# NWC-CUAHSI-Summer-Institute/LGAR-py

Hardware: AMD Instinct MI355X
Metric: column-timesteps/sec (higher is better)
Workload: dtype f32

## Files before the change

lgar_py_amd/csrc/lgar_column.hpp:

```cpp
#pragma once
#include "lgar_geff.hpp"

namespace lgar {

template <typename R> struct Glob {
  R dt_h, initial_psi, pdm, wp_psi, frozen;
  R giuh[LGAR_GMAX];
  int nint, nsub, ng, bottom_mode, closed_form;
  long long iter_cap;
};

#define LGAR_COOP_GROUPS 16
template <typename S, int FMAX, int STRIDE = WAVE> struct FrontsView {
  S *base;
  unsigned char *fl;
  __device__ __forceinline__ S &Z(int i) const { return base[(0 * FMAX + i) * STRIDE]; }
  __device__ __forceinline__ S &TH(int i) const { return base[(1 * FMAX + i) * STRIDE]; }
  __device__ __forceinline__ S &PS(int i) const { return base[(2 * FMAX + i) * STRIDE]; }
  __device__ __forceinline__ S &DZ(int i) const { return base[(3 * FMAX + i) * STRIDE]; }
  __device__ __forceinline__ unsigned char &flag(int i) const { return fl[i * STRIDE]; }
  __device__ __forceinline__ int layer(int i) const { return fl[i * STRIDE] & 0x7f; }
  __device__ __forceinline__ bool bottom(int i) const { return (fl[i * STRIDE] & LGAR_FLAG_BOTTOM) != 0; }
  __device__ __forceinline__ void set_flag(int i, int layer, bool bottom) const {
    fl[i * STRIDE] = (unsigned char)(layer | (bottom ? LGAR_FLAG_BOTTOM : 0));
  }
  __device__ __forceinline__ void copy(int dst, int src) const {
    Z(dst) = Z(src); TH(dst) = TH(src); PS(dst) = PS(src); DZ(dst) = DZ(src);
    fl[dst * STRIDE] = fl[src * STRIDE];
  }
};

constexpr int MODE_LITERAL = 0, MODE_FAST = 1, MODE_MIXED = 3, MODE_COOP = 4, MODE_MIXED_COOP = 6;

template <typename S, int MODE> struct ModeTraits : ScalarKind<S> {
  using K = ScalarKind<S>;
  static constexpr bool literal = MODE == MODE_LITERAL;
  static constexpr bool mixed = MODE == MODE_MIXED || MODE == MODE_MIXED_COOP;
  static constexpr bool coop = MODE == MODE_COOP || MODE == MODE_MIXED_COOP;
  static constexpr bool mixed_f64 = mixed && K::plain_f64;
  static constexpr bool coop_f64 = coop && K::plain_f64;
  static constexpr int pol = (literal && K::f64) ? POL_LIBRARY : (!literal && K::plain_f32) ? POL_RCP32 : mixed_f64 ? POL_MIXED : POL_LEAN;
  static constexpr int stride = coop ? LGAR_COOP_GROUPS : WAVE;
  static constexpr bool giuh_mem = MODE == MODE_MIXED && !K::dual;
  static constexpr bool late_forcing_sums = MODE == MODE_MIXED;
  static constexpr bool fused_walk = !literal && !coop;
};

template <typename S, int NL, int FMAX, int MODE> struct Column {
  using R = real_t<S>;
  using M = ModeTraits<S, MODE>;
  static constexpr int POL = M::pol;
  const ColParams<S, NL> &P;
  const LGAR_KARG Glob<R> *G;
  FrontsView<S, FMAX, M::stride> F;
  int nf;
  int status;
  S ponded_water, previous_precip, ending_volume;
  S giuh_q[LGAR_GMAX];
  static constexpr int DEAD = LGAR_ST_BOTTOM | LGAR_ST_OVERFLOW | LGAR_ST_STRUCT;
  R *giuh_mem = nullptr;
  size_t giuh_stride = 0;
  bool giuh_live = false;
  S k_deepest;
  bool new_front_frozen;
  S memo_theta, memo_g;
  int memo_layer = -1;
  unsigned near_sat_fronts = 0u;
  S post_mass;
  bool post_mass_valid = false;
  bool post_event = false;
  bool psi_rewritten = false;
  S aet_psi_wp_memo;
  bool aet_psi_wp_known = false;
  bool count_geff = false;
  int share_lanes = 0;
  R *xchg = nullptr;
  int coop_rank = 0;
  int cap = FMAX;
  S a_precip, a_pet, a_aet, a_infil, a_runoff, a_perc, a_giuh, a_disch;

  __device__ Column(const ColParams<S, NL> &p, const LGAR_KARG Glob<R> *g, const FrontsView<S, FMAX, M::stride> &f) : P(p), G(g), F(f) {}

  __device__ __forceinline__ S cum_at(int k) const { return sel<S, NL>(P.cum, k); }
  __device__ __forceinline__ S capillary_drive(const LayerK<S> &lk, S theta1, S theta2, int site = 0, CoopRiders *riders = nullptr) {
    (void)site; (void)riders;
    LGAR_MEASURE_POINT(NOGEFF, lk, theta1, theta2)
    LGAR_COUNT_GEFF_CALL(site)
    LGAR_MEASURE_POINT(DUP_GEFF, lk, theta1, theta2)
    if constexpr (M::literal && M::f64) {
      return G->closed_form ? geff_closed<S, POL>(lk, theta1, theta2) : geff_literal<S, POL>(lk, theta1, theta2, G->nint);
    }
    if constexpr (M::dual && M::f64 && !M::literal) {
      if (share_lanes >= 2 && !G->closed_form) return geff_fused<S>(lk, theta1, theta2, G->nint, xchg, share_lanes);
    }
    if constexpr (M::coop_f64 && !M::mixed) {
      if (share_lanes > 1 && !G->closed_form) return geff_fused<S>(lk, theta1, theta2, G->nint, xchg, share_lanes, coop_rank, riders);
    }
    if constexpr (M::coop_f64 && M::mixed) {
      if (share_lanes > 1 && !G->closed_form)
        return geff_mixed_coop(val(lk.alpha), val(lk.n), val(lk.m), val(lk.inv_m), val(lk.inv_n), val(lk.ksat), val(lk.te), val(lk.tr),
                               theta1, theta2, G->nint, xchg, share_lanes, coop_rank);
    }
    if constexpr (M::mixed_f64) {
      if (!G->closed_form)
        return geff_mixed(val(lk.alpha), val(lk.n), val(lk.m), val(lk.inv_m), val(lk.inv_n), val(lk.ksat), val(lk.te), val(lk.tr),
                          theta1, theta2, G->nint);
    }
#ifndef LGAR_NO_F32_RARE_GEFF
    if constexpr (M::plain_f32 && !M::literal) {
      if (site != 1 && !G->closed_form)
        return geff_f32_rare(lk.alpha, lk.n, lk.m, lk.inv_m, lk.inv_n, lk.te, lk.tr, theta1, theta2, G->nint);
    }
#endif
    return G->closed_form ? geff_closed<S, POL>(lk, theta1, theta2) : geff(lk, theta1, theta2, G->nint);
  }
  __device__ __forceinline__ double capillary_drive_fronts(const LayerK<double> &lk, double theta1, double theta2, double psi1,
                                                           double psi2, double &kr_end) {
    LGAR_MEASURE_POINT(NOGEFF_FRONTS, lk, theta1, theta2, kr_end)
    LGAR_COUNT_GEFF_CALL(1)
    if constexpr (M::coop && M::mixed) {
      if (share_lanes > 1) return geff_mixed_heads<true>(lk, theta1, theta2, psi1, psi2, G->nint, kr_end, xchg, share_lanes, coop_rank);
    }
    return geff_mixed_heads(lk, theta1, theta2, psi1, psi2, G->nint, kr_end);
  }
  __device__ __forceinline__ S cum_prev(int k) const {
    S r = S(R(0.0));
#pragma unroll
// ... 1016 lines not shown
      const LayerK<S> lk = pick(P, k);
      LGAR_COUNT_GEFF_CALL(1)
      LGAR_COUNT_GEFF_CALL(1)
      double kr_mine;
      const S g_mine = geff_mixed_heads<true>(lk, F.TH(im + 1), F.TH(im), F.PS(im + 1), F.PS(im), G->nint, kr_mine, tab2, hl, r2);
      tab2[0] = g_mine;
      tab2[1] = kr_mine;
#pragma unroll
      for (int j = 0; j < NL - 1; j++)
        if (j < kmax) {
          const LayerK<S> lj = pick_static(P, j);
          const S tl = theta_from_h<S, POL>(lj, F.PS(im));
          tab2[2 + j] = k_from_se<S, POL>(lj, se_from_theta(lj, tl));
        }
      lds_exchange_point();
      S g2[2];
      R kr2[2], kk[2][NL];
#pragma unroll
      for (int h = 0; h < 2; h++) {
        g2[h] = xchg[h * 64];
        kr2[h] = xchg[h * 64 + 1];
#pragma unroll
        for (int j = 0; j < NL - 1; j++) kk[h][j] = xchg[h * 64 + 2 + j];
      }
      lds_exchange_point();
#pragma unroll
      for (int h = 0; h < 2; h++) {
        const int f = h ? ib : ia;
        const int kf = h ? kb : ka;
        const LayerK<S> lf = pick(P, kf);
        const S g = g2[h];
        S ki = lf.ksat * kr2[h];
        if (f == 0 && new_front_frozen) ki = ki * G->frozen;
        if (is_nan(val(g))) status |= LGAR_ST_NAN;
        const S delta_theta = F.TH(f) - F.TH(f + 1);
        S dzdt;
        if (kf == 0) {
          dzdt = dv<POL>(S(R(1.0)), delta_theta) * (dv<POL>(lf.ksat * (g + h_p), F.Z(f)) + ki);
        } else {
          S den = S(R(0.0)) + dv<POL>(F.Z(f) - cum_prev(kf), ki);
#pragma unroll
          for (int j = 0; j < NL - 1; j++)
            if (j < kf) {
              S pt = (j != 0) ? P.cum[(j > 0) ? j - 1 : 0] : S(R(0.0));
              den = den + dv<POL>(P.cum[j] - pt, S(kk[h][j]));
            }
          dzdt = dv<POL>(S(R(1.0)), delta_theta) * (dv<POL>(F.Z(f), den) + dv<POL>(lf.ksat * (g + h_p), F.Z(f)));
        }
        F.DZ(f) = dzdt;
      }
    }
  }

  __device__ __forceinline__ void calc_dzdt(S h_p) {
    int i = -1;
    if constexpr (M::coop_f64 && M::mixed) {
      if (share_lanes >= 4 && !G->closed_form) i = calc_dzdt_pairs_mixed(h_p);
    }
    if constexpr (M::coop_f64 && !M::mixed) {
      if (share_lanes >= LGAR_COOP_PAIR_LANES && !G->closed_form) i = calc_dzdt_pairs(h_p);
    }
    for (;;) {
      bool found = false;
      while (!found && ++i < nf - 1) {
        if (F.bottom(i)) { F.DZ(i) = S(R(0.0)); continue; }
        const bool top = F.layer(i) == 0;
        if (top && val(F.TH(i + 1)) > val(F.TH(i))) status |= LGAR_ST_THETA_ORDER;
        if (val(F.TH(i) - F.TH(i + 1)) > R(0.0)) found = true;
        else F.DZ(i) = S(R(0.0));
      }
      if (any_lane(found) == 0ull) break;
      LGAR_MEASURE_POINT(CLK, 10)
      if (found) {
        const int k = F.layer(i);
        const LayerK<S> lk = pick(P, k);
        S theta_1 = F.TH(i + 1), theta_2 = F.TH(i);
        S delta_theta = F.TH(i) - F.TH(i + 1);
        S g, ki;
        bool fronts_done = false;
        if constexpr (M::mixed_f64) {
          if (!G->closed_form) {
            double kr_end;
            g = capillary_drive_fronts(lk, theta_1, theta_2, F.PS(i + 1), F.PS(i), kr_end);
            ki = lk.ksat * kr_end;
            if (i == 0 && new_front_frozen) ki = ki * G->frozen;
            fronts_done = true;
          }
        }
        CoopRiders riders;
        if constexpr (M::coop_f64 && !M::mixed) {
          if (!G->closed_form && share_lanes >= 5 + k) {
            const int e = coop_rank - 5;
            LayerK<S> le = lk;
            S th_e = F.TH(i);
            if (k > 0) {
#pragma unroll
              for (int j = 0; j < NL - 1; j++) {
                const bool mine = (e == j) && (j < k);
                le.alpha = choose(mine, P.alpha[j], le.alpha); le.n = choose(mine, P.n[j], le.n); le.m = choose(mine, P.m[j], le.m);
                le.inv_m = choose(mine, P.inv_m[j], le.inv_m); le.ksat = choose(mine, P.ksat[j], le.ksat);
                le.te = choose(mine, P.te[j], le.te); le.tr = choose(mine, P.tr[j], le.tr);
              }
              const S tl = theta_from_h<S, POL>(le, F.PS(i));
              th_e = choose(e >= 0 && e < k, tl, th_e);
            }
            riders.n = 1 + k;
            riders.l = le;
            riders.se = se_from_theta(le, th_e);
#pragma unroll
            for (int q = 0; q < LGAR_LMAX; q++) riders.k[q] = R(1.0);
            g = capillary_drive(lk, theta_1, theta_2, 1, &riders);
            ki = riders.k[0];
            if (i == 0 && new_front_frozen) ki = ki * G->frozen;
            fronts_done = true;
          }
        }
        LGAR_MEASURE_POINT(F32_HEADS_FROM_PSI, lk, i, g, ki, fronts_done)
        if (!fronts_done) {
          g = capillary_drive(lk, theta_1, theta_2, 1);
          ki = front_k(i, lk);
#ifndef LGAR_NO_DZDT_MEMO
          if constexpr (M::plain_f32 && !M::literal) {
            if (same_bits(theta_2, lk.te) && (i == 0 || F.layer(i - 1) != k)) { memo_theta = theta_1; memo_g = g; memo_layer = k; }
          }
#endif
        }
        if (is_nan(val(g))) status |= LGAR_ST_NAN;
        S dzdt;
        if (k == 0) {
          dzdt = dv<POL>(S(R(1.0)), delta_theta) * (dv<POL>(lk.ksat * (g + h_p), F.Z(i)) + ki);
        } else {
          S den = S(R(0.0)) + dv<POL>(F.Z(i) - cum_prev(k), ki);
#pragma unroll
          for (int j = 0; j < NL - 1; j++)
            if (j < k) {
              const LayerK<S> lj = pick_static(P, j);
              S kl;
              bool rode = false;
              if constexpr (M::coop_f64 && !M::mixed) {
                if (riders.n > 0) { kl = riders.k[1 + j]; rode = true; }
              }
              if (!rode) {
                S tl = theta_from_h<S, POL>(lj, F.PS(i));
                kl = k_from_se<S, POL>(lj, se_from_theta(lj, tl));
              }
              S pt = (j != 0) ? P.cum[(j > 0) ? j - 1 : 0] : S(R(0.0));
              den = den + dv<POL>(P.cum[j] - pt, kl);
            }
          dzdt = dv<POL>(S(R(1.0)), delta_theta) * (dv<POL>(F.Z(i), den) + dv<POL>(lk.ksat * (g + h_p), F.Z(i)));
        }
        F.DZ(i) = dzdt;
        LGAR_MEASURE_POINT(CLK, 17)
      }
    }
  }

  __device__ __forceinline__ S calc_dry_depth() {
    const LayerK<S> l0 = pick_static(P, 0);
    S delta_theta = l0.te - F.TH(0);
    S tau = G->dt_h * l0.ksat / delta_theta;
    S g = capillary_drive(l0, F.TH(0), l0.te, 2);
    if (is_nan(val(g))) status |= LGAR_ST_NAN;
    S dry = R(0.5) * (tau + sq(tau * tau + R(4.0) * tau * g));
    return mn(P.cum[0], dry);
  }

  __device__ __forceinline__ void create_surficial_front(S dry_depth, S &ponded, S &infiltration) {
    if (nf >= cap) { status |= LGAR_ST_OVERFLOW; return; }
    const LayerK<S> l0 = pick_static(P, 0);
    S cur_theta = F.TH(0);
    S delta_theta = l0.te - cur_theta;
    S theta_new;
    bool to_bottom = false;
    if (val(dry_depth * delta_theta) > val(ponded)) {
      infiltration = ponded;
      theta_new = mn((cur_theta + ponded / dry_depth), l0.te);
      ponded = S(R(0.0));
    } else {
      infiltration = dry_depth * delta_theta;
      ponded = ponded - (dry_depth * delta_theta);
      theta_new = l0.te;
      to_bottom = !(val(dry_depth) < val(P.cum[0]));
    }
    for (int j = nf; j > 0; j--) F.copy(j, j - 1);
    nf++;
    F.Z(0) = dry_depth;
    F.TH(0) = theta_new;
    F.set_flag(0, 0, to_bottom);
    F.PS(0) = h_from_se<S, POL>(l0, se_from_theta(l0, theta_new));
    new_front_frozen = true;
    F.DZ(0) = S(R(0.0));
  }

  __device__ __forceinline__ void insert_water(int fdd, S precip, S &ponded, S &infiltration, S &runoff) {
    const R dt = G->dt_h;
    S h_p = (ponded - precip) * dt;
    if (val(h_p) < R(0.0)) h_p = S(R(0.0));
    const int kfp = F.layer(fdd);
    int lo, len;
    range_of(kfp, lo, len);
    const int nxt_i = lo + 1;
    if (nxt_i >= nf && (nf != NL || G->bottom_mode == 0)) { status |= LGAR_ST_STRUCT; return; }
    const LayerK<S> lk = pick(P, kfp);
    S g = S(R(0.0));
    if (nf != NL) {
      const S theta_1 = F.TH(nxt_i < nf ? nxt_i : nf - 1);
      bool hit = memo_layer == kfp && same_bits(theta_1, memo_theta);
      if constexpr (M::dual) {
        if (share_lanes >= 2) {
          const bool value_hit = memo_layer == kfp && val(theta_1) == val(memo_theta);
          if (any_lane(value_hit && !hit) != 0ull) hit = false;
        }
      }
      if (hit) {
        g = memo_g;
      } else {
        g = capillary_drive(lk, theta_1, lk.te, 3);
        memo_theta = theta_1; memo_g = g; memo_layer = kfp;
      }
    }
    if (is_nan(val(g))) status |= LGAR_ST_NAN | LGAR_ST_NEGBASE;
    S f_p;
    if (kfp == 0) {
      f_p = P.ksat[0] * (R(1.0) + dv<POL>(g + h_p, F.Z(fdd)));
    } else {
      S fd_ksat = lk.ksat * G->frozen;
      S bottom_sum = dv<POL>(F.Z(fdd) - cum_prev(kfp), fd_ksat);
      bottom_sum = bottom_sum + dv<POL>(P.cum[0] - R(0.0), P.ksat[0] * G->frozen);
#pragma unroll
      for (int j = 1; j < NL - 1; j++)
        if (j < kfp) {
          const LayerK<S> lj = pick_static(P, j);
          S tl = theta_from_h<S, POL>(lj, F.PS(fdd));
          S kl = k_from_se<S, POL>(lj, se_from_theta(lj, tl));
          bottom_sum = bottom_sum + dv<POL>(P.cum[j] - P.cum[j - 1], kl);
        }
      f_p = dv<POL>(F.Z(fdd), bottom_sum) + dv<POL>((g + h_p) * fd_ksat, F.Z(fdd));
    }
    S pond_temp = ponded - f_p * dt;
    if (val(pond_temp) < R(0.0)) pond_temp = S(R(0.0));
    S fp_cm = f_p * dt;
    if (G->pdm > R(0.0)) {
      if (val(pond_temp) < G->pdm) {
        infiltration = mn(ponded, fp_cm);
        ponded = ponded - infiltration;
      } else if (val(pond_temp) > G->pdm) {
        ponded = S(G->pdm);
        infiltration = fp_cm;
      }
      S r = pond_temp - G->pdm;
      runoff = (val(r) > R(0.0)) ? r : S(R(0.0));
    } else {
      infiltration = mn(ponded, fp_cm);
      S r = ponded - infiltration;
      ponded = S(G->pdm);
      runoff = (val(r) > R(0.0)) ? r : S(R(0.0));
    }
  }

  __device__ __forceinline__ void init_state() {
    nf = NL;
    status = 0;
    new_front_frozen = false;
#pragma unroll
    for (int k = 0; k < NL; k++) {
      const LayerK<S> lk = pick_static(P, k);
      F.Z(k) = P.cum[k];
      F.TH(k) = theta_from_h<S, POL>(lk, S(G->initial_psi));
      F.PS(k) = S(G->initial_psi);
      if (k == NL - 1) k_deepest = k_from_se<S, POL>(lk, se_from_theta(lk, F.TH(k)));
      F.DZ(k) = S(R(0.0));
      F.set_flag(k, k, true);
    }
    ponded_water = previous_precip = S(R(0.0));
#pragma unroll
    for (int i = 0; i < LGAR_GMAX; i++) giuh_q[i] = S(R(0.0));
    ending_volume = mass_balance();
    drain();
  }

  __device__ __forceinline__ void drain() {
    a_precip = a_pet = a_aet = a_infil = a_runoff = a_perc = a_giuh = a_disch = S(R(0.0));
  }

  __device__ __forceinline__ void forward(S precip, S pet) {
    const R dt = G->dt_h;
    if (is_nan(val(precip)) || is_nan(val(pet))) status |= LGAR_ST_NAN;
    S ending_volume_sub = ending_volume;
    for (int sub = 0; sub < G->nsub; sub++) {
      if (status & DEAD) return;
      new_front_frozen = false;
      post_mass_valid = false;
      S precip_sub = precip * dt;
      S pet_sub = pet * dt;
      S ponded_depth_sub = precip_sub + ponded_water;
      S ponded_water_sub = S(R(0.0)), runoff_sub = S(R(0.0)), infiltration_sub = S(R(0.0)), AET_sub = S(R(0.0));
      const bool create = (val(previous_precip) == R(0.0)) && (val(precip_sub) > R(0.0)) && (val(ponded_water) == R(0.0));
      LGAR_MEASURE_POINT(CLK, 0)
      LGAR_MEASURE_POINT(DUP_FDD)
      const int fdd = free_drainage_front();
      const bool saturated = val(F.TH(0)) >= val(P.te[0]);
      if (val(pet) > R(0.0)) {
        if (!aet_psi_wp_known) {
          aet_psi_wp_memo = aet_psi_wp<S, POL>(pick_static(P, 0), G->wp_psi);
          aet_psi_wp_known = true;
        }
        AET_sub = aet_from_psi_wp<S, POL>(pet, dt, F.PS(0), aet_psi_wp_memo);
      }
      if constexpr (!M::late_forcing_sums) {
        a_precip = a_precip + precip_sub;
        a_pet = a_pet + ((val(pet_sub) > R(0.0)) ? pet_sub : S(R(0.0)));
      }
      const bool inserting = !create && val(ponded_depth_sub) > R(0.0);
      LGAR_MEASURE_POINT(CLK, 1)
      if (inserting) {
        LGAR_ABLATABLE(INSERT, insert_water(fdd, precip_sub, ponded_depth_sub, infiltration_sub, runoff_sub);)
        a_infil = a_infil + infiltration_sub;
        a_runoff = a_runoff + runoff_sub;
        ponded_water_sub = ponded_depth_sub;
      }
      LGAR_MEASURE_POINT(CLK, 2)
      if (!create || !saturated) {
        S perc_sub = S(R(0.0));
        LGAR_ABLATABLE(MOVE, perc_sub = move_wetting_front(create ? S(R(0.0)) : infiltration_sub, AET_sub, ending_volume_sub, fdd);)
        if (!create) a_perc = a_perc + perc_sub;
      }
      if (__builtin_expect(create && !saturated, 0)) {
        S dry_depth = calc_dry_depth();
        create_surficial_front(dry_depth, ponded_depth_sub, infiltration_sub);
        a_infil = a_infil + infiltration_sub;
        post_mass_valid = false;
      }
      if (!inserting) {
        if (val(ponded_depth_sub) < G->pdm) {
          runoff_sub = S(R(0.0));
          ponded_water_sub = ponded_depth_sub;
          ponded_depth_sub = S(R(0.0));
        } else {
          runoff_sub = ponded_depth_sub - G->pdm;
          ponded_depth_sub = S(G->pdm);
          ponded_water_sub = ponded_depth_sub;
          a_runoff = a_runoff + runoff_sub;
        }
      }
      LGAR_MEASURE_POINT(CLK, 5)
      LGAR_ABLATABLE(DZDT, calc_dzdt(ponded_depth_sub);)
      LGAR_MEASURE_POINT(CLK, 6)
      LGAR_MEASURE_POINT(DUP_DZDT, ponded_depth_sub)
      LGAR_MEASURE_POINT(DUP_MB, ending_volume_sub)
      if constexpr (M::fused_walk) {
        if (__builtin_expect(!post_mass_valid, 0)) post_mass = mass_balance();
        ending_volume_sub = post_mass;
      } else {
        ending_volume_sub = mass_balance();
      }
      LGAR_MEASURE_POINT(CLK, 7)
      previous_precip = precip_sub;
      ending_volume = ending_volume_sub;
      if constexpr (M::late_forcing_sums) {
        a_precip = a_precip + precip_sub;
        a_pet = a_pet + ((val(pet_sub) > R(0.0)) ? pet_sub : S(R(0.0)));
      }
      a_aet = a_aet + AET_sub;
      ponded_water = ponded_water_sub;
      if constexpr (M::giuh_mem) {
        if (giuh_live || val(runoff_sub) > R(0.0)) {
          const int ng = G->ng;
          S q[LGAR_GMAX];
#pragma unroll
// ... 44 lines not shown
```

lgar_py_amd/csrc/lgar_forward_body.hpp:

```cpp
#pragma once
#include "lgar_column.hpp"

namespace lgar {

template <typename R> struct KArgs {
  int N, T, F;
  int Nf, Fg;
  int coop;
  unsigned *ticket;
  int chain_first, chain_last;
  const unsigned *pending_in;
  unsigned *pending_out;
  const R *alpha, *n, *ksat, *theta_e, *theta_r, *thick;
  R *depth, *theta, *psi, *k, *dzdt;
  uint8_t *flags;
  int32_t *nf;
  R *scalars;
  R *totals;
  const R *precip, *pet;
  R *series[LGAR_NACC];
  double *basin;
  const R *weights;
  unsigned basin_mask;
  int32_t *status;
// ... 262 lines not shown
    bool active = (t >= t_begin) && (t < t_stop_at.get());
    if (active && !a.chain_last && col.nf + a.G.nsub > FMAX) {
      active = false;
      t_stop_at.set(t);
    }
    if (any_lane(active) == 0ull) continue;
    if (active) col.forward(precip, pet);
    LGAR_MEASURE_POINT(BALLAST_TOUCH)
    if constexpr (AHEAD) {
      settle_load(precip_ahead);
      settle_load(pet_ahead);
    }
    const R acc[LGAR_NACC] = {col.a_precip, col.a_pet, col.a_aet, col.a_infil, col.a_runoff,
                              col.a_perc, col.a_giuh, col.a_disch, col.ponded_water, col.ending_volume};
    if (active && leader) {
#pragma unroll
      for (int j = 0; j < LGAR_NACC; j++)
        if (series_mask & (1u << j)) a.series[j][o] = acc[j];
    }
    LGAR_MEASURE_POINT(CLK, 18)
    if (basin_on) {
      const double w = active ? wgt : 0.0;
#pragma unroll
      for (int j = 0; j < LGAR_NACC; j++)
        if (a.basin_mask & (1u << j)) {
          const double s = wave_sum(w * (double)acc[j]);
          if (lane == 0) {
            if constexpr (PARK) atomic_add_uniform(&a.basin[(size_t)j * T + t], s);
            else atomic_add(&a.basin[(size_t)j * T + t], s);
          }
        }
    }
    if (active) {
#pragma unroll
      for (int j = 0; j < 7; j++) {
        if (j == 5 && a.G.bottom_mode == 0) continue;
        const int row = sum_row<SR>(j);
        if (row >= 0) lds.sums[row][slot] = lds.sums[row][slot] + acc[j];
        else tot[j] = tot[j] + acc[j];
      }
      col.drain();
    }
    LGAR_MEASURE_POINT(CLK, 21)
  }
  LGAR_MEASURE_POINT(BALLAST_FOLD, col)
  ap = launder(ap);
  const LGAR_KARG KArgs<R> &z = *ap;
  if (z.counters != nullptr) {
    const double calls = wave_sum((double)((unsigned)col.status >> LGAR_ST_STEP_SHIFT));
    if (lane == 0 && calls > 0.0) {
      if constexpr (PARK) atomic_add_uniform(&z.counters[0], (unsigned long long)calls);
      else atomic_add(&z.counters[0], (unsigned long long)calls);
    }
  }
  col.status &= LGAR_ST_FAULT_MASK;
  const int t_stop = t_stop_at.get();
  if (t_begin >= z.T) return;
  if (!leader) return;
  if (z.pending_out != nullptr) {
    const unsigned long long m = any_lane(t_stop >= 0 && t_stop < z.T);
    if (m != 0ull && first_active_lane()) {
      if constexpr (PARK) atomic_add_uniform(z.pending_out, (unsigned)__builtin_popcountll(m));
      else atomic_add(z.pending_out, (unsigned)__builtin_popcountll(m));
    }
  }
  int word = col.status;
  if (t_stop >= 0 && t_stop < z.T) word |= LGAR_ST_RESUME | (int)((unsigned)t_stop << LGAR_ST_STEP_SHIFT);
  if (t_stop <= t_begin) {
    z.status[c] = word;
    if (z.call_sums != nullptr && z.chain_first) {
#pragma unroll
      for (int j = 0; j < 8; j++) z.call_sums[j * N + c] = R(0);
      z.call_sums[8 * N + c] = col.ponded_water;
      z.call_sums[9 * N + c] = col.ending_volume;
    }
    return;
  }
  store_state<R, NL, FMAX, MODE>(z, c, col, nf_before, word);
#pragma unroll
  for (int j = 0; j < 7; j++)
    if (sum_row<SR>(j) >= 0) tot[j] = lds.sums[sum_row<SR>(j)][slot];
  tot[7] = tot[6];
#pragma unroll
  for (int j = 0; j < 8; j++) z.totals[j * N + c] = z.totals[j * N + c] + tot[j];
  z.totals[8 * N + c] = col.ponded_water;
  z.totals[9 * N + c] = col.ending_volume;
  if (z.call_sums != nullptr) {
    const bool add = !z.chain_first;
#pragma unroll
    for (int j = 0; j < 8; j++) z.call_sums[j * N + c] = add ? z.call_sums[j * N + c] + tot[j] : tot[j];
    z.call_sums[8 * N + c] = col.ponded_water;
    z.call_sums[9 * N + c] = col.ending_volume;
  }
}

}
```

lgar_py_amd/csrc/lgar_geff.hpp:

```cpp
#pragma once
#include "lgar_vg.hpp"

namespace lgar {

#define LGAR_COOP_TAB 128
#define LGAR_COOP_TAB_ROW 130
#define LGAR_COOP_PAIR_LANES 12
#ifndef LGAR_DEVSIM
template <int W>
__device__ __forceinline__ void geff_coop_node_rounds(const LayerK<double> &l, double nm1, double half_m, double k_sat1, double k_first,
                                                      double hdh, int nint, int lanes, double *tab, int r) {
  const int stride = W * lanes;
  for (int first = 0; first < nint; first += stride) {
    double h[W], k[W];
    bool ok[W];
#pragma unroll
    for (int u = 0; u < W; u++) {
      const int j = first + r + u * lanes;
      ok[u] = (r < lanes) && (j < nint);
      h[u] = tab[ok[u] ? j : 0];
    }
#pragma unroll
    for (int u = 0; u < W; u++) k[u] = geff_node(l, nm1, half_m, h[u]);
#pragma unroll
// ... 283 lines not shown
    const f32x2 t = __builtin_elementwise_fma(-P, (SR) * (SR), one2);          \
    (TT) = t * t;                                                              \
  }
  int it = 0;
  for (; it + 1 < safe_pairs; it += 2) {
    const f32x2 xa = __builtin_elementwise_fma(ja, dx2, x02);
    const f32x2 xb = __builtin_elementwise_fma(ja + two2, dx2, x02);
    ja = ja + four2;
    f32x2 sa, ta, sb, tb;
    LGAR_GEFF_PAIR(xa, sa, ta)
    acc = __builtin_elementwise_fma(sa, ta, acc);
    LGAR_GEFF_PAIR(xb, sb, tb)
    accb = __builtin_elementwise_fma(sb, tb, accb);
  }
  if (it < safe_pairs) {
    const f32x2 x = __builtin_elementwise_fma(ja, dx2, x02);
    f32x2 sr, tt;
    LGAR_GEFF_PAIR(x, sr, tt)
    acc = __builtin_elementwise_fma(sr, tt, acc);
    it++;
  }
  for (; it < pairs; it++) {
    const float j0 = float(2 * it + 1);
    const f32x2 j2 = {j0, j0 + 1.0f};
    const f32x2 x = __builtin_elementwise_fma(j2, dx2, x02);
    f32x2 sr, tt;
    LGAR_GEFF_PAIR(x, sr, tt)
    sr.x = (x.x < xcut) ? ksat1 : sr.x;
    tt.x = (x.x < xcut) ? 1.0f : tt.x;
    sr.y = (x.y < xcut) ? ksat1 : sr.y;
    tt.y = (x.y < xcut) ? 1.0f : tt.y;
    if (it & 1) accb = __builtin_elementwise_fma(sr, tt, accb);
    else acc = __builtin_elementwise_fma(sr, tt, acc);
  }
  acc = acc + accb;
  float sum = acc.x + acc.y;
  if (M & 1) sum += node(__builtin_fmaf(float(M), dx, x0));
#ifndef LGAR_NO_GEFF_ENDS
  float k0, kn;
  {
    const f32x2 xe = {x0, l.alpha * h_f};
    f32x2 sr, tt;
    LGAR_GEFF_PAIR(xe, sr, tt)
    sr.x = (xe.x < xcut) ? ksat1 : sr.x;
    tt.x = (xe.x < xcut) ? 1.0f : tt.x;
    sr.y = (xe.y < xcut) ? ksat1 : sr.y;
    tt.y = (xe.y < xcut) ? 1.0f : tt.y;
    const f32x2 ke = sr * tt;
    k0 = ke.x; kn = ke.y;
  }
#else
  const float k0 = node(x0), kn = node(l.alpha * h_f);
#endif
#undef LGAR_GEFF_PAIR
  if (kn_out != nullptr) *kn_out = kn;
  return fabsf((0.5f * dh) * ((k0 + kn) + 2.0f * sum));
}
template <> __device__ __forceinline__ float geff<float>(const LayerK<float> &l, float theta1, float theta2, int nint) {
  const float se_i = se_from_theta(l, theta1);
  const float se_f = se_from_theta(l, theta2);
  const float inv_alpha = 1.0f / l.alpha;
#ifndef LGAR_NO_GEFF_ENDS
  const float ni = -l.inv_m;
  const float la = lg2(se_i), lb = lg2(se_f);
  const float pa = ex2(ni * la), pb = ex2(ni * lb);
  float ba = pa - 1.0f, bb = pb - 1.0f;
  if (fabsf(ba) <= 1e-8f) ba = ba + 1e-12f;
  if (fabsf(bb) <= 1e-8f) bb = bb + 1e-12f;
  const float ua = lg2(ba), ub = lg2(bb);
  const float oa = ex2(l.inv_n * ua), ob = ex2(l.inv_n * ub);
  return geff_f32_from_heads(l, inv_alpha * oa, inv_alpha * ob, nint);
#else
  auto head = [&](float se) {
    float base = pw(se, -l.inv_m) - 1.0f;
    if (fabsf(base) <= 1e-8f) base = base + 1e-12f;
    return inv_alpha * pw(base, l.inv_n);
  };
  return geff_f32_from_heads(l, head(se_i), head(se_f), nint);
#endif
}
__device__ __attribute__((noinline)) float geff_f32_rare(float alpha, float n, float m, float inv_m, float inv_n, float te, float tr,
                                                         float theta1, float theta2, int nint) {
  const LayerK<float> l{alpha, n, m, inv_m, inv_n, 1.0f, te, tr};
  return geff<float>(l, theta1, theta2, nint);
}
template <> __device__ __forceinline__ double geff<double>(const LayerK<double> &l, double t1, double t2, int nint) {
  return geff_fused<double>(l, t1, t2, nint);
}

#define LGAR_LOG2_1EM12 -39.863137138648355
__device__ __forceinline__ void mixed_end(const LayerK<double> &l, double se, double &h, double &kr) {
  const double q = lg2e(se) * l.inv_m;
  const double C = ex2e(q);
  const double omc = 1.0 - C;
  const bool k_nudged = fabs(omc) <= 1e-8;
  const double bk = k_nudged ? omc + 1e-12 : omc;
  const double u = (omc == 0.0) ? LGAR_LOG2_1EM12 : lg2e(bk);
  const double t = 1.0 - ex2e(l.m * u);
  kr = sqrt(se) * (t * t);
  const double bh = omc / C;
  const bool h_nudged = fabs(bh) <= 1e-8;
  double lbh = (omc == 0.0) ? u : u - q;
  if (any_lane((k_nudged || h_nudged) && omc != 0.0) != 0ull) {
    const double own = lg2e(h_nudged ? bh + 1e-12 : bh);
    lbh = ((k_nudged || h_nudged) && omc != 0.0) ? own : lbh;
  }
  h = (1.0 / l.alpha) * ex2e(lbh * l.inv_n);
}
template <bool COOPERATE = false>
__device__ __forceinline__ double geff_mixed_core(const LayerK<double> &l, double h_i, double h_f, double k0, double kn_own, double ksat1,
                                                  int nint, double *tab = nullptr, int lanes = 0, int r = 0) {
  (void)tab; (void)lanes; (void)r;
  const float ksat1f = (float)ksat1;
  const double dh = (h_f - h_i) / double(nint);
  const double x0 = l.alpha * h_i, dx = l.alpha * dh, xcut = 0.1 * l.alpha;
  const double hmd = -0.5 * l.m;
  const float hm = (float)hmd, hm_lo = (float)(hmd - (double)hm);
  const int M = nint - 1;
  const int pairs = M >> 1;
  const double inv_ndx = 1.0 / -dx;
  const double jf = (x0 - xcut) * inv_ndx - 1.5;
  int safe = (jf > 0.0) ? ((jf < double(M)) ? int(jf) : M) : 0;
  safe >>= 1;
  int safe_pairs = pairs;
  if (!COOPERATE && any_lane(safe < pairs) != 0ull) {
    safe_pairs = 0;
    for (int bit = 64; bit; bit >>= 1) {
      const int cand = safe_pairs + bit;
      if (cand <= pairs && any_lane(safe < cand) == 0ull) safe_pairs = cand;
    }
  }
  const float xcutf = (float)xcut;
  const float nf = (float)l.n, nf_lo = (float)(l.n - (double)nf), mmf = (float)(-l.m), mmf_lo = (float)(-l.m - (double)mmf);
  const f32x2 n2 = {nf, nf}, nl2 = {nf_lo, nf_lo}, hm2 = {hm, hm}, hml2 = {hm_lo, hm_lo}, one2 = {1.0f, 1.0f};
  const f32x2 ln2_2 = {0.693147181f, 0.693147181f}, c2_2 = {0.240226507f, 0.240226507f}, c3_2 = {0.0555041087f, 0.0555041087f};
  const f32x2 c4_2 = {0.00961812911f, 0.00961812911f}, c5_2 = {0.00133335581f, 0.00133335581f};
  const f32x2 mm2 = {mmf, mmf}, mml2 = {mmf_lo, mmf_lo}, ilog2 = {1.44269504f, 1.44269504f}, two_ilog2 = {2.88539008f, 2.88539008f};
  const f32x2 half2 = {0.5f, 0.5f};
// ... 253 lines not shown
```

lgar_py_amd/csrc/lgar_measure.hpp:

```cpp
#pragma once
#ifdef LGAR_NO_F32_REUSE
#define LGAR_NO_DZDT_MEMO
#define LGAR_NO_F32_RARE_GEFF
#define LGAR_NO_GEFF_ENDS
#endif

__device__ __forceinline__ float opaque(float x) { asm volatile("" : "+v"(x)); return x; }
__device__ __forceinline__ double opaque(double x) { asm volatile("" : "+v"(x)); return x; }

#define LGAR_MEASURE_POINT(NAME, ...) LGAR_POINT_##NAME(__VA_ARGS__)
#define LGAR_ABLATABLE(NAME, ...) LGAR_STMT_##NAME(__VA_ARGS__)

#ifdef LGAR_ABL_NOINSERT
#define LGAR_STMT_INSERT(...)
#else
#define LGAR_STMT_INSERT(...) __VA_ARGS__
#endif
#ifdef LGAR_ABL_NOMOVE
#define LGAR_STMT_MOVE(...)
#else
#define LGAR_STMT_MOVE(...) __VA_ARGS__
#endif
#ifdef LGAR_ABL_NODZDT
#define LGAR_STMT_DZDT(...)
#else
#define LGAR_STMT_DZDT(...) __VA_ARGS__
#endif

#ifdef LGAR_ABL_NOGEFF
#define LGAR_POINT_NOGEFF(lk, theta1, theta2) return theta1 * theta2 + lk.alpha;
#else
#define LGAR_POINT_NOGEFF(lk, theta1, theta2)
#endif
#ifdef LGAR_ABL_NOGEFF
#define LGAR_POINT_NOGEFF_FRONTS(lk, theta1, theta2, kr) { kr = theta1; return theta1 * theta2 + lk.alpha; }
#else
#define LGAR_POINT_NOGEFF_FRONTS(lk, theta1, theta2, kr)
#endif
#ifdef LGAR_COUNT_SITE
#define LGAR_COUNT_IF_SITE(site) if (site == LGAR_COUNT_SITE)
#else
#define LGAR_COUNT_IF_SITE(site)
#endif
#ifdef LGAR_COUNT_MAXLANES
#define LGAR_COUNT_IF_SPARSE if (__builtin_popcountll(any_lane(true)) <= LGAR_COUNT_MAXLANES)
#else
#define LGAR_COUNT_IF_SPARSE
#endif
#ifdef LGAR_COUNT_LANES
#define LGAR_COUNT_WHO count_geff
#else
#define LGAR_COUNT_WHO (count_geff && first_active_lane())
#endif
#define LGAR_COUNT_GEFF_CALL(site) \
  LGAR_COUNT_IF_SITE(site) LGAR_COUNT_IF_SPARSE { if (LGAR_COUNT_WHO) status += (1 << LGAR_ST_STEP_SHIFT); }
#ifdef LGAR_DUP_GEFF
#define LGAR_POINT_DUP_GEFF(lk, theta1, theta2)                                                    \
// ... 141 lines not shown
```

lgar_py_amd/engine.py:

```python
import ctypes as C

import torch

from . import _capi
from ._capi import ACC_NAMES, GMAX, LMAX, LMIN, NACC, NSCAL, LgarError

BASIN_SCRATCH_BYTES = 8 << 30
PARAMS = ("alpha", "n", "ksat", "theta_e", "theta_r", "thickness")
SETTINGS = dict(dt_h=1.0, num_subcycles=1, initial_psi=2000.0, ponded_depth_max=0.0, wilting_point_psi=15495.0,
                frozen_factor=1.0, nint=120, giuh_ordinates=(0.06, 0.51, 0.28, 0.12, 0.03), dtype=torch.float64,
                device="cuda:0", iter_cap=0, search_mode=1, bottom_mode=0, use_closed_form_G=False, front_slots=None,
                geff_precision="native", forward_lanes=0, basin_scratch_bytes=BASIN_SCRATCH_BYTES)
_DIMS_SETTINGS = ("dt_h", "num_subcycles", "initial_psi", "ponded_depth_max", "wilting_point_psi", "frozen_factor", "nint",
                  "giuh_ordinates", "iter_cap", "search_mode", "bottom_mode", "use_closed_form_G", "forward_lanes")


def _require_gpu(device):
    if not torch.cuda.is_available():
        raise LgarError("no ROCm GPU visible: the LGAR engine has no CPU fallback (device=%s)" % (device,))


def _ptr(t):
    return None if t is None else t.data_ptr()

# ... 204 lines not shown
            st["d_in"].copy_(h_in, non_blocking=True)
            _capi.check(self.lib.lgar_forward(*st["args"], self._dt, C.c_void_p(stream.cuda_stream)), "lgar_forward")
            st["h_out"].copy_(st["d_out"], non_blocking=True)
            st["h_status"].copy_(self.status, non_blocking=True)
            stream.synchronize()
        return st["h_out"][:NACC], st["h_out"][NACC], st["h_out"][NACC + 1], st["h_status"]

    def raise_for_status(self, status_host):
        if bool((status_host != 0).any()):
            self.check_status()

    def tangent(self, direction, precip, pet, w_runoff=None, w_perc=None, want_series=False, forcing_group=1, share=0):
        prep = lambda t: None if t is None else torch.as_tensor(t).to(self.device, self.dtype).contiguous()
        precip, pet = self._forcing(precip, pet, forcing_group)
        w_runoff, w_perc = prep(w_runoff), prep(w_perc)
        share = int(share)
        if share != 0 and (not 2 <= share <= 32 or self.N % share != 0):
            raise LgarError("share must be 0 or 2..32 (with n_columns a multiple of it)")
        if share:
            for t in (self.alpha, self.n, self.ksat, self.theta_e, self.theta_r, self.thickness):
                gw = t.reshape(t.shape[0], -1, share)
                if not bool((gw == gw[:, :, :1]).all()):
                    raise LgarError("share=%d needs identical soil parameters within each group of %d columns" % (share, share))
            if forcing_group % share != 0 and precip.shape[1] != 1:
                raise LgarError("share=%d needs the columns of a group to read the same forcing column (forcing_group a "
                                "multiple of it, or one forcing column for all)" % share)
        self.dims.tangent_share = int(share)
        for nm, w in (("w_runoff", w_runoff), ("w_perc", w_perc)):
            if w is not None and w.shape != precip.shape:
                raise LgarError("%s must be [T, N] like the forcing; got %s" % (nm, tuple(w.shape)))
        T = precip.shape[0]
        dirs = {k: prep(direction.get(k)) for k in ("alpha", "n", "ksat")}
        for k, v in dirs.items():
            if v is not None and tuple(v.shape) != (self.L, self.N):
                raise LgarError("direction[%r] must be [L, N]" % k)
        dstruct = _capi.LgarParams(_ptr(dirs["alpha"]), _ptr(dirs["n"]), _ptr(dirs["ksat"]), None, None, None)
        grad = torch.zeros(self.N, dtype=self.dtype, device=self.device)
        ser = self._new_series(T, self.N, dtype=self.dtype, device=self.device) if want_series else None
        st = torch.zeros(self.N, dtype=torch.int32, device=self.device)
        tickets = torch.zeros(_capi.NTICKETS, dtype=torch.int32, device=self.device)
        fo = _capi.LgarForcing(precip.data_ptr(), pet.data_ptr())
        self._call("forward_tangent", C.byref(self.dims), C.byref(self._params), C.byref(dstruct), C.byref(fo), _ptr(w_runoff),
                   _ptr(w_perc), grad.data_ptr(), _ptr(ser), st.data_ptr(), counters=tickets)
        return grad, ser, st

    def cooperating_lanes(self):
        return int(self.lib.lgar_cooperating_lanes(C.byref(self.dims), self._dt))

    def geff_wave_calls(self, reset=True):
        n = int(self.counters[0].item())
        if reset:
            self.counters.zero_()
        return n

    def check_status(self):
        st = self.status
        if not bool((st != 0).any()):
            return
        bad = torch.nonzero(st)[:, 0]
        kinds = torch.tensor(list(_capi.STATUS_NAMES), dtype=st.dtype, device=st.device)
        present = ((st[bad, None] & kinds) != 0).any(0).tolist()
        names = [nm for nm, there in zip(_capi.STATUS_NAMES.values(), present) if there]
        raise LgarStatusError("%d of %d columns faulted (%s); first column %d, max status %d"
                              % (bad.numel(), self.N, ", ".join(names), int(bad[0].item()), int(st.max().item())))

    def fronts(self):
        fl = self.flags.cpu().numpy()
        return dict(depth=self.depth.cpu().numpy(), theta=self.theta.cpu().numpy(), psi=self.psi.cpu().numpy(),
                    k=self.k.cpu().numpy(), dzdt=self.dzdt.cpu().numpy(), layer=(fl & 0x7F).astype("int8"),
                    to_bottom=(fl >> 7).astype("int8"), n_fronts=self.n_fronts.cpu().numpy())

    def _moisture_bins(self, edges, what):
        self._need_state()
        if what not in _capi.MOIST_WHAT:
            raise LgarError("what must be 'theta' or 'storage' (got %r)" % (what,))
        if edges is None:
            return None, self.L
        try:
            e = torch.as_tensor(edges).detach().to("cpu", torch.float64)
        except (TypeError, ValueError, RuntimeError) as err:
            raise LgarError("edges must be a 1-D sequence of depths in cm (%s)" % err)
        if e.dim() != 1 or e.numel() < 2:
            raise LgarError("edges must be 1-D with at least two entries (got shape %s)" % (tuple(e.shape),))
        if e.numel() - 1 > _capi.MOIST_BINS:
            raise LgarError("at most %d bins (LGAR_MOIST_BINS); got %d" % (_capi.MOIST_BINS, e.numel() - 1))
        if not bool(torch.isfinite(e).all()) or float(e[0]) < 0.0 or not bool((e[1:] > e[:-1]).all()):
            raise LgarError("edges must be finite, >= 0 and strictly increasing")
        return e.to(self.device).contiguous(), e.numel() - 1

    def _moisture_launch(self, e_dev, n_bins, what, out, w, sums):
        self._call("soil_moisture", C.byref(self.dims), C.byref(self._params), C.byref(self._state), _ptr(e_dev), n_bins,
                   _capi.MOIST_WHAT[what], out.data_ptr(), _ptr(w), _ptr(sums))

    def _moisture_weights(self, weights):
        if weights is None:
            return None
        w = torch.as_tensor(weights).to(self.device, self.dtype).contiguous()
        if tuple(w.shape) != (self.N,):
            raise LgarError("weights must be [N]")
        return w

    def soil_moisture(self, edges=None, what="theta", out=None, weights=None, basin=False):
        e_dev, D = self._moisture_bins(edges, what)
        if out is None:
            out = torch.empty(D, self.N, dtype=self.dtype, device=self.device)
        elif (not isinstance(out, torch.Tensor) or tuple(out.shape) != (D, self.N) or out.dtype != self.dtype
# ... 95 lines not shown
```

Measured before the change: 12.70 billion.

## Split Green-Ampt integral across idle wave lanes and read dzdt memo

Adds a wave-cooperative f32 capillary-drive (Geff) path: lanes that need an integral are paired with idle lanes via ds_permute, and each pair sums the even and odd quadrature nodes. This applies in calc_dzdt and insert_water, and only when idle lanes are at least as many as needy ones. calc_dzdt also reuses a memoized Geff when theta matches the cached value. The aim is to cut divergent serial integral cost within a wave, at the price of extra cross-lane shuffles, ballots, a noinline call, and a restructured insert_water split into open/miss/close stages.

```diff
diff --git a/lgar_py_amd/csrc/lgar_column.hpp b/lgar_py_amd/csrc/lgar_column.hpp
--- a/lgar_py_amd/csrc/lgar_column.hpp
+++ b/lgar_py_amd/csrc/lgar_column.hpp
@@ -73,6 +73,7 @@
   S aet_psi_wp_memo;
   bool aet_psi_wp_known = false;
   bool count_geff = false;
+  int geff_shared_calls = 0;
   int share_lanes = 0;
   R *xchg = nullptr;
   int coop_rank = 0;
@@ -1195,6 +1196,54 @@
     }
   }
 
+  __device__ __forceinline__ bool known_or_shared_geff(int i, bool found, S &g) {
+    bool known = false, need = found;
+    S alpha = S(R(1.0)), n = S(R(2.0)), m = S(R(0.5)), inv_m = S(R(2.0)), inv_n = S(R(0.5)), te = S(R(1.0)), tr = S(R(0.0));
+    S theta_1 = S(R(0.5)), theta_2 = S(R(1.0));
+    if (found) {
+      const int k = F.layer(i);
+      const LayerK<S> lk = pick(P, k);
+      alpha = lk.alpha; n = lk.n; m = lk.m; inv_m = lk.inv_m; inv_n = lk.inv_n; te = lk.te; tr = lk.tr;
+      theta_1 = F.TH(i + 1); theta_2 = F.TH(i);
+#ifndef LGAR_NO_DZDT_MEMO_READ
+      if (same_bits(theta_2, lk.te) && (i == 0 || F.layer(i - 1) != k) && memo_layer == k && same_bits(theta_1, memo_theta)) {
+        g = memo_g;
+        known = true;
+        need = false;
+      }
+#endif
+    }
+#ifndef LGAR_NO_GEFF_SPLIT
+    const unsigned long long need_m = any_lane(need);
+    if (need_m != 0ull) {
+      const unsigned long long idle_m = any_lane(true) & ~need_m;
+#ifdef LGAR_GEFF_SPLIT_SELF
+      const bool share = true;
+#else
+      const bool share = __builtin_popcountll(need_m) <= __builtin_popcountll(idle_m);
+#endif
+      if (share) {
+        const S gs = geff_shared(alpha, n, m, inv_m, inv_n, te, tr, theta_1, theta_2, need, 1);
+        if (need) { g = gs; known = true; }
+      }
+    }
+#endif
+    return known;
+  }
+#ifndef LGAR_NO_GEFF_SPLIT
+  __device__ __forceinline__ S geff_shared(S alpha, S n, S m, S inv_m, S inv_n, S te, S tr, S theta_1, S theta_2, bool need, int site) {
+    (void)site;
+    if constexpr (M::plain_f32 && !M::literal) {
+      if (need) {
+        LGAR_COUNT_GEFF_CALL(site)
+        if (count_geff && first_active_lane()) geff_shared_calls++;
+      }
+      return geff_f32_shared(alpha, n, m, inv_m, inv_n, te, tr, theta_1, theta_2, G->nint, need);
+    }
+    return S(R(0.0));
+  }
+#endif
+
   __device__ __forceinline__ void calc_dzdt(S h_p) {
     int i = -1;
     if constexpr (M::coop_f64 && M::mixed) {
@@ -1214,6 +1263,11 @@
       }
       if (any_lane(found) == 0ull) break;
       LGAR_MEASURE_POINT(CLK, 10)
+      S g_known = S(R(0.0));
+      bool g_is_known = false;
+      if constexpr (M::plain_f32 && !M::literal) {
+        if (!G->closed_form) g_is_known = known_or_shared_geff(i, found, g_known);
+      }
       if (found) {
         const int k = F.layer(i);
         const LayerK<S> lk = pick(P, k);
@@ -1260,7 +1314,8 @@
         }
         LGAR_MEASURE_POINT(F32_HEADS_FROM_PSI, lk, i, g, ki, fronts_done)
         if (!fronts_done) {
-          g = capillary_drive(lk, theta_1, theta_2, 1);
+          if (g_is_known) g = g_known;
+          else g = capillary_drive(lk, theta_1, theta_2, 1);
           ki = front_k(i, lk);
 #ifndef LGAR_NO_DZDT_MEMO
           if constexpr (M::plain_f32 && !M::literal) {
@@ -1335,16 +1390,60 @@
     F.DZ(0) = S(R(0.0));
   }
 
+  struct InsertWater {
+    int kfp = 0;
+    LayerK<S> lk{S(R(1.0)), S(R(2.0)), S(R(0.5)), S(R(2.0)), S(R(0.5)), S(R(1.0)), S(R(1.0)), S(R(0.0))};
+    S theta_1 = S(R(0.5)), h_p = S(R(0.0)), g = S(R(0.0));
+    bool miss = false;
+  };
   __device__ __forceinline__ void insert_water(int fdd, S precip, S &ponded, S &infiltration, S &runoff) {
+    InsertWater w;
+    if (!insert_water_open(fdd, precip, ponded, w)) return;
+    if (w.miss) insert_water_miss(w, capillary_drive(w.lk, w.theta_1, w.lk.te, 3));
+    insert_water_close(fdd, w, ponded, infiltration, runoff);
+  }
+  __device__ __forceinline__ void insert_water_miss(InsertWater &w, S g) {
+    w.g = g;
+    w.miss = false;
+    memo_theta = w.theta_1; memo_g = g; memo_layer = w.kfp;
+  }
+#ifndef LGAR_NO_GEFF_SPLIT
+  __device__ __forceinline__ void insert_water_wave(int fdd, bool inserting, S precip, S &ponded, S &infiltration, S &runoff) {
+    InsertWater w;
+    bool go = false;
+    if (inserting) go = insert_water_open(fdd, precip, ponded, w);
+    if (!G->closed_form) {
+      const unsigned long long need_m = any_lane(w.miss);
+      if (need_m != 0ull) {
+#ifdef LGAR_GEFF_SPLIT_SELF
+        const bool share = true;
+#else
+        const bool share = __builtin_popcountll(need_m) <= __builtin_popcountll(any_lane(true) & ~need_m);
+#endif
+        if (share) {
+          const S gs = geff_shared(w.lk.alpha, w.lk.n, w.lk.m, w.lk.inv_m, w.lk.inv_n, w.lk.te, w.lk.tr, w.theta_1, w.lk.te, w.miss, 3);
+          if (w.miss) insert_water_miss(w, gs);
+        }
+      }
+    }
+    if (!go) return;
+    if (w.miss) insert_water_miss(w, capillary_drive(w.lk, w.theta_1, w.lk.te, 3));
+    insert_water_close(fdd, w, ponded, infiltration, runoff);
+  }
+#endif
+  __device__ __forceinline__ bool insert_water_open(int fdd, S precip, const S &ponded, InsertWater &w) {
     const R dt = G->dt_h;
     S h_p = (ponded - precip) * dt;
     if (val(h_p) < R(0.0)) h_p = S(R(0.0));
+    w.h_p = h_p;
     const int kfp = F.layer(fdd);
+    w.kfp = kfp;
     int lo, len;
     range_of(kfp, lo, len);
     const int nxt_i = lo + 1;
-    if (nxt_i >= nf && (nf != NL || G->bottom_mode == 0)) { status |= LGAR_ST_STRUCT; return; }
-    const LayerK<S> lk = pick(P, kfp);
+    if (nxt_i >= nf && (nf != NL || G->bottom_mode == 0)) { status |= LGAR_ST_STRUCT; return false; }
+    w.lk = pick(P, kfp);
+    const LayerK<S> &lk = w.lk;
     S g = S(R(0.0));
     if (nf != NL) {
       const S theta_1 = F.TH(nxt_i < nf ? nxt_i : nf - 1);
@@ -1355,13 +1454,18 @@
           if (any_lane(value_hit && !hit) != 0ull) hit = false;
         }
       }
-      if (hit) {
-        g = memo_g;
-      } else {
-        g = capillary_drive(lk, theta_1, lk.te, 3);
-        memo_theta = theta_1; memo_g = g; memo_layer = kfp;
-      }
-    }
+      w.theta_1 = theta_1;
+      if (hit) g = memo_g;
+      else w.miss = true;
+    }
+    w.g = g;
+    return true;
+  }
+  __device__ __forceinline__ void insert_water_close(int fdd, const InsertWater &w, S &ponded, S &infiltration, S &runoff) {
+    const R dt = G->dt_h;
+    const int kfp = w.kfp;
+    const LayerK<S> &lk = w.lk;
+    const S g = w.g, h_p = w.h_p;
     if (is_nan(val(g))) status |= LGAR_ST_NAN | LGAR_ST_NEGBASE;
     S f_p;
     if (kfp == 0) {
@@ -1456,8 +1560,15 @@
       }
       const bool inserting = !create && val(ponded_depth_sub) > R(0.0);
       LGAR_MEASURE_POINT(CLK, 1)
+#ifndef LGAR_NO_GEFF_SPLIT
+      if constexpr (M::plain_f32 && !M::literal) {
+        LGAR_ABLATABLE(INSERT, insert_water_wave(fdd, inserting, precip_sub, ponded_depth_sub, infiltration_sub, runoff_sub);)
+      } else
+#endif
       if (inserting) {
         LGAR_ABLATABLE(INSERT, insert_water(fdd, precip_sub, ponded_depth_sub, infiltration_sub, runoff_sub);)
+      }
+      if (inserting) {
         a_infil = a_infil + infiltration_sub;
         a_runoff = a_runoff + runoff_sub;
         ponded_water_sub = ponded_depth_sub;
diff --git a/lgar_py_amd/csrc/lgar_forward_body.hpp b/lgar_py_amd/csrc/lgar_forward_body.hpp
--- a/lgar_py_amd/csrc/lgar_forward_body.hpp
+++ b/lgar_py_amd/csrc/lgar_forward_body.hpp
@@ -338,6 +338,10 @@
       if constexpr (PARK) atomic_add_uniform(&z.counters[0], (unsigned long long)calls);
       else atomic_add(&z.counters[0], (unsigned long long)calls);
     }
+    if constexpr (M::plain_f32 && !M::literal) {
+      const double shared = wave_sum((double)col.geff_shared_calls);
+      if (lane == 0 && shared > 0.0) atomic_add(&z.counters[1], (unsigned long long)shared);
+    }
   }
   col.status &= LGAR_ST_FAULT_MASK;
   const int t_stop = t_stop_at.get();
diff --git a/lgar_py_amd/csrc/lgar_geff.hpp b/lgar_py_amd/csrc/lgar_geff.hpp
--- a/lgar_py_amd/csrc/lgar_geff.hpp
+++ b/lgar_py_amd/csrc/lgar_geff.hpp
@@ -359,7 +359,6 @@
 #else
   const float k0 = node(x0), kn = node(l.alpha * h_f);
 #endif
-#undef LGAR_GEFF_PAIR
   if (kn_out != nullptr) *kn_out = kn;
   return fabsf((0.5f * dh) * ((k0 + kn) + 2.0f * sum));
 }
@@ -391,6 +390,181 @@
   const LayerK<float> l{alpha, n, m, inv_m, inv_n, 1.0f, te, tr};
   return geff<float>(l, theta1, theta2, nint);
 }
+#ifndef LGAR_NO_GEFF_SPLIT
+__device__ __forceinline__ f32x2 geff_f32_parity_sum(float x0, float dx, float nm1, float hm, float xcut, float ksat1, int nint, int par,
+                                                     bool mine) {
+  const int M = nint - 1;
+  const int pairs = M >> 1;
+#ifndef LGAR_DEVSIM
+  const float jf = (x0 - xcut) * __builtin_amdgcn_rcpf(-dx) - 1.5f;
+#else
+  const float jf = (x0 - xcut) / -dx - 1.5f;
+#endif
+  int safe = (jf > 0.0f) ? ((jf < float(M)) ? int(jf) : M) : 0;
+  safe = mine ? (safe >> 1) : pairs;
+  int safe_pairs = pairs;
+  if (any_lane(safe < pairs) != 0ull) {
+    safe_pairs = 0;
+    for (int bit = 64; bit; bit >>= 1) {
+      const int cand = safe_pairs + bit;
+      if (cand <= pairs && any_lane(safe < cand) == 0ull) safe_pairs = cand;
+    }
+  }
+  const int nq = pairs >> 1;
+  const int sq = safe_pairs >> 1;
+  const f32x2 dx2 = {dx, dx}, x02 = {x0, x0}, nm12 = {nm1, nm1}, hm2 = {hm, hm};
+  const f32x2 one2 = {1.0f, 1.0f}, four2 = {4.0f, 4.0f}, eight2 = {8.0f, 8.0f};
+  const float j00 = float(2 * par + 1);
+  f32x2 ja = {j00, j00 + 1.0f};
+  f32x2 acc = {0.0f, 0.0f};
+  int q = 0;
+  for (; q + 1 < sq; q += 2) {
+    const f32x2 xa = __builtin_elementwise_fma(ja, dx2, x02);
+    const f32x2 xb = __builtin_elementwise_fma(ja + four2, dx2, x02);
+    ja = ja + eight2;
+    f32x2 sa, ta, sb, tb;
+    LGAR_GEFF_PAIR(xa, sa, ta)
+    LGAR_GEFF_PAIR(xb, sb, tb)
+    acc = __builtin_elementwise_fma(sa, ta, acc);
+    acc = __builtin_elementwise_fma(sb, tb, acc);
+  }
+  for (; q < nq; q++) {
+    const float j0 = float(4 * q + 1) + float(2 * par);
+    const f32x2 j2 = {j0, j0 + 1.0f};
+    const f32x2 x = __builtin_elementwise_fma(j2, dx2, x02);
+    f32x2 sr, tt;
+    LGAR_GEFF_PAIR(x, sr, tt)
+    sr.x = (x.x < xcut) ? ksat1 : sr.x;
+    tt.x = (x.x < xcut) ? 1.0f : tt.x;
+    sr.y = (x.y < xcut) ? ksat1 : sr.y;
+    tt.y = (x.y < xcut) ? 1.0f : tt.y;
+    acc = __builtin_elementwise_fma(sr, tt, acc);
+  }
+  return acc;
+}
+__device__ __attribute__((noinline)) float geff_f32_shared(float alpha, float n, float m, float inv_m, float inv_n, float te, float tr,
+                                                           float theta1, float theta2, int nint, bool need) {
+  const LayerK<float> l{alpha, n, m, inv_m, inv_n, 1.0f, te, tr};
+  const float se_i = se_from_theta(l, theta1);
+  const float se_f = se_from_theta(l, theta2);
+  const float inv_alpha = 1.0f / l.alpha;
+#ifndef LGAR_NO_GEFF_ENDS
+  const float ni = -l.inv_m;
+  const float la = lg2(se_i), lb = lg2(se_f);
+  const float pa = ex2(ni * la), pb = ex2(ni * lb);
+  float ba = pa - 1.0f, bb = pb - 1.0f;
+  if (fabsf(ba) <= 1e-8f) ba = ba + 1e-12f;
+  if (fabsf(bb) <= 1e-8f) bb = bb + 1e-12f;
+  const float ua = lg2(ba), ub = lg2(bb);
+  const float oa = ex2(l.inv_n * ua), ob = ex2(l.inv_n * ub);
+  const float h_i = inv_alpha * oa, h_f = inv_alpha * ob;
+#else
+  auto head = [&](float se) {
+    float base = pw(se, -l.inv_m) - 1.0f;
+    if (fabsf(base) <= 1e-8f) base = base + 1e-12f;
+    return inv_alpha * pw(base, l.inv_n);
+  };
+  const float h_i = head(se_i), h_f = head(se_f);
+#endif
+  const float dh = (h_f - h_i) * (1.0f / float(nint));
+  float nm1 = l.n - 1.0f;
+  float hm = -0.5f * l.m;
+  float x0 = l.alpha * h_i, dx = l.alpha * dh, xcut = 0.1f * l.alpha;
+  const float tsat = 1.0f - ex2(l.m * -39.863137f);
+  float ksat1 = tsat * tsat;
+  const int M = nint - 1;
+  const int pairs = M >> 1;
+  f32x2 acc, accb;
+#ifndef LGAR_DEVSIM
+  const unsigned long long need_m = any_lane(need);
+  unsigned long long nm = need_m, im = any_lane(true) & ~need_m;
+  const int lane = (int)(threadIdx.x & 63u);
+  int partner = lane;
+  if ((nm | im) == ~0ull) {
+    const int owners = __builtin_popcountll(nm);
+    const int rn = (int)__builtin_amdgcn_mbcnt_hi((unsigned)(nm >> 32), __builtin_amdgcn_mbcnt_lo((unsigned)nm, 0u));
+    const int ri = (int)__builtin_amdgcn_mbcnt_hi((unsigned)(im >> 32), __builtin_amdgcn_mbcnt_lo((unsigned)im, 0u));
+    const int held = __builtin_amdgcn_ds_permute((need ? rn : 63 - ri) << 2, lane);
+    const int found = __builtin_amdgcn_ds_bpermute((need ? 63 - rn : ri) << 2, held);
+    partner = (need || ri < owners) ? found : lane;
+  } else {
+    while (nm != 0ull && im != 0ull) {
+      const int a = __builtin_ctzll(nm), b = __builtin_ctzll(im);
+      nm &= nm - 1ull;
+      im &= im - 1ull;
+      partner = (lane == a) ? b : ((lane == b) ? a : partner);
+    }
+  }
+  const bool helper = !need && partner != lane;
+  {
+    const float x0p = __shfl(x0, partner), dxp = __shfl(dx, partner), nm1p = __shfl(nm1, partner), hmp = __shfl(hm, partner);
+    const float xcutp = __shfl(xcut, partner), ksat1p = __shfl(ksat1, partner);
+    x0 = helper ? x0p : x0; dx = helper ? dxp : dx; nm1 = helper ? nm1p : nm1; hm = helper ? hmp : hm;
+    xcut = helper ? xcutp : xcut; ksat1 = helper ? ksat1p : ksat1;
+  }
+  acc = geff_f32_parity_sum(x0, dx, nm1, hm, xcut, ksat1, nint, helper ? 1 : 0, need || helper);
+  accb.x = __shfl(acc.x, partner);
+  accb.y = __shfl(acc.y, partner);
+#else
+  acc = geff_f32_parity_sum(x0, dx, nm1, hm, xcut, ksat1, nint, 0, true);
+  accb = geff_f32_parity_sum(x0, dx, nm1, hm, xcut, ksat1, nint, 1, true);
+#endif
+  const f32x2 dx2 = {dx, dx}, x02 = {x0, x0}, nm12 = {nm1, nm1}, hm2 = {hm, hm}, one2 = {1.0f, 1.0f};
+  if (pairs & 1) {
+    const float j0 = float(2 * pairs - 1);
+    const f32x2 j2 = {j0, j0 + 1.0f};
+    const f32x2 x = __builtin_elementwise_fma(j2, dx2, x02);
+    f32x2 sr, tt;
+    LGAR_GEFF_PAIR(x, sr, tt)
+    sr.x = (x.x < xcut) ? ksat1 : sr.x;
+    tt.x = (x.x < xcut) ? 1.0f : tt.x;
+    sr.y = (x.y < xcut) ? ksat1 : sr.y;
+    tt.y = (x.y < xcut) ? 1.0f : tt.y;
+    acc = __builtin_elementwise_fma(sr, tt, acc);
+  }
+  acc = acc + accb;
+  float sum = acc.x + acc.y;
+  if (M & 1) {
+    const float x = __builtin_fmaf(float(M), dx, x0);
+    const float lg = lg2(x);
+    const float P = ex2(nm1 * lg);
+    const float l1 = lg2(__builtin_fmaf(x, P, 1.0f));
+    const float sr = ex2(hm * l1);
+    const float t = __builtin_fmaf(-P, sr * sr, 1.0f);
+    const float k = sr * (t * t);
+    sum += (x < xcut) ? ksat1 : k;
+  }
+  float k0, kn;
+#ifndef LGAR_NO_GEFF_ENDS
+  {
+    const f32x2 xe = {x0, l.alpha * h_f};
+    f32x2 sr, tt;
+    LGAR_GEFF_PAIR(xe, sr, tt)
+    sr.x = (xe.x < xcut) ? ksat1 : sr.x;
+    tt.x = (xe.x < xcut) ? 1.0f : tt.x;
+    sr.y = (xe.y < xcut) ? ksat1 : sr.y;
+    tt.y = (xe.y < xcut) ? 1.0f : tt.y;
+    const f32x2 ke = sr * tt;
+    k0 = ke.x; kn = ke.y;
+  }
+#else
+  {
+    auto node = [&](float x) {
+      const float lg = lg2(x);
+      const float P = ex2(nm1 * lg);
+      const float l1 = lg2(__builtin_fmaf(x, P, 1.0f));
+      const float sr = ex2(hm * l1);
+      const float t = __builtin_fmaf(-P, sr * sr, 1.0f);
+      const float k = sr * (t * t);
+      return (x < xcut) ? ksat1 : k;
+    };
+    k0 = node(x0); kn = node(l.alpha * h_f);
+  }
+#endif
+  return fabsf((0.5f * dh) * ((k0 + kn) + 2.0f * sum));
+}
+#endif
+#undef LGAR_GEFF_PAIR
 template <> __device__ __forceinline__ double geff<double>(const LayerK<double> &l, double t1, double t2, int nint) {
   return geff_fused<double>(l, t1, t2, nint);
 }
diff --git a/lgar_py_amd/csrc/lgar_measure.hpp b/lgar_py_amd/csrc/lgar_measure.hpp
--- a/lgar_py_amd/csrc/lgar_measure.hpp
+++ b/lgar_py_amd/csrc/lgar_measure.hpp
@@ -3,6 +3,8 @@
 #define LGAR_NO_DZDT_MEMO
 #define LGAR_NO_F32_RARE_GEFF
 #define LGAR_NO_GEFF_ENDS
+#define LGAR_NO_DZDT_MEMO_READ
+#define LGAR_NO_GEFF_SPLIT
 #endif
 
 __device__ __forceinline__ float opaque(float x) { asm volatile("" : "+v"(x)); return x; }
diff --git a/lgar_py_amd/engine.py b/lgar_py_amd/engine.py
--- a/lgar_py_amd/engine.py
+++ b/lgar_py_amd/engine.py
@@ -280,6 +280,9 @@
         if reset:
             self.counters.zero_()
         return n
+
+    def geff_shared_calls(self):
+        return int(self.counters[1].item())
 
     def check_status(self):
         st = self.status
```

New measurement: 12.82 billion (median of 6 runs). No clear change (+1.0%).
